# JaredWinkens/sdr-iq-visualizer

Measured on AMD Instinct MI355X. Metric: complex64 IQ Msamples/s through windowed FFT+log-PSD, N=4096; % HBM3E peak, higher is better.
Workload: dtype f32

## Files before the change

### sdr-iq-visualizer_amd/csrc/fft4096.hip

```cpp
#include "fft4096_core.h"

namespace sdrk {

template <bool HAS_WINDOW, int EPILOGUE>
__global__ __launch_bounds__(F4K_THREADS, F4K_WAVES) void fft4096_kernel(
    const float2* __restrict__ iq, size_t frame_stride, void* __restrict__ out_raw,
    size_t n_frames, const float* __restrict__ window, const float2* __restrict__ tw4096,
    float eps, int shift) {
    typedef F4kInC64 In;
    __shared__ float2 lds[f4k_lds_elems(HAS_WINDOW)];
    float2* __restrict__ tw256 = lds + F4K_XCH_ELEMS;
    float2* __restrict__ tw1 = tw256 + 256;
    float* __restrict__ lds_win = reinterpret_cast<float*>(tw1 + 256);

    const int tid = threadIdx.x;
    F4kAddr A = f4k_addr(tid);
    f4k_init_tables(tw256, tw1, tw4096, tid);
    if (HAS_WINDOW) {
#pragma unroll
        for (int j = 0; j < 16; ++j) lds_win[tid + 256 * j] = window[tid + 256 * j];
    }
    __syncthreads();

    const int xor_k2 = shift ? 8 : 0;
    constexpr int OUT_ELEM = (EPILOGUE == EPI_LOGPSD ? 4 : 8);
    const int voff_out = tid * OUT_ELEM;

    const size_t first = blockIdx.x;
    const size_t step = gridDim.x;

    auto issue = [&](In::word (&x)[16], size_t fr) {
        if (fr >= n_frames) fr = first;
        In::issue(x, iq + fr * frame_stride, tid);
    };
    auto process = [&](In::word (&x)[16], size_t f) {
        In::to_owners(x, lds, tid);
        cf v[16];
#pragma unroll
        for (int j = 0; j < 16; ++j) v[j] = In::widen(x[j]);
        issue(x, f + step);
        f4k_windowed_transform<HAS_WINDOW>(v, lds, tw256, tw1, lds_win, A, tid);
        f4k_store_row<EPILOGUE>(v, frame_rsrc(static_cast<char*>(out_raw) + f * (size_t)(F4K_N * OUT_ELEM), F4K_N * OUT_ELEM),
                                voff_out, xor_k2, eps);
    };
    In::word nxt[16];
    issue(nxt, first);
    for (size_t f = first; f < n_frames; f += step) process(nxt, f);
}

hipError_t launch_fft4096(const LaunchArgs& a) {
    if (a.n_frames == 0) return hipSuccess;
    dim3 g(f4k_grid(a.num_cus, F4K_WAVES, a.n_frames)), b(F4K_THREADS);
    const float2* iq = static_cast<const float2*>(a.d_iq);
    const float2* tw = static_cast<const float2*>(a.d_twiddle);
#define SDRK_LAUNCH(W, E)                                                                            \
    hipLaunchKernelGGL((fft4096_kernel<W, E>), g, b, 0, a.stream, iq, a.frame_stride, a.d_out,           \
                       a.n_frames, a.d_window, tw, a.eps, a.shift)
    if (a.epilogue == EPI_LOGPSD) {
        if (a.d_window) SDRK_LAUNCH(true, EPI_LOGPSD); else SDRK_LAUNCH(false, EPI_LOGPSD);
    } else {
        if (a.d_window) SDRK_LAUNCH(true, EPI_COMPLEX); else SDRK_LAUNCH(false, EPI_COMPLEX);
    }
#undef SDRK_LAUNCH
    return hipGetLastError();
}

}
```

### sdr-iq-visualizer_amd/csrc/kernels.h

```cpp
#pragma once
#include <hip/hip_runtime.h>
#include <stddef.h>
#include <stdint.h>

#include <atomic>

#ifdef SDRK_PHASE_MARKS
#define SDRK_PHASE(name) asm volatile("; SDRK_PHASE " name ::: "memory")
#else
#define SDRK_PHASE(name) do { } while (0)
#endif

namespace sdrk {

enum Epilogue : int {
    EPI_LOGPSD = 0,
    EPI_COMPLEX = 1,
    EPI_BLU_MUL = 2,
    EPI_BLU_POST_LOG = 3,
    EPI_BLU_POST_C64 = 4,
};

struct LaunchArgs {
    const void* d_iq = nullptr;
    size_t frame_stride = 0;
    void* d_out = nullptr;
    size_t n_frames = 0;
    int nfft = 0;
    const float* d_window = nullptr;
    const void* d_twiddle = nullptr;
    float eps = 1e-12f;
    int shift = 1;
    int epilogue = EPI_LOGPSD;
    hipStream_t stream = nullptr;
    int num_cus = 256;
    void* d_scratch = nullptr;
    size_t scratch_frames = 0;
    const void* d_twiddle_2p = nullptr;
    hipStream_t stream2 = nullptr;
    hipEvent_t ev_col[2] = {nullptr, nullptr}, ev_row[2] = {nullptr, nullptr}, ev_fork = nullptr;
    int col_cus = 0, row_cus = 0;
    float* d_mip = nullptr;
    bool* mip_written = nullptr;
    const float2* d_epi_tab = nullptr;
    int epi_n_out = 0;
    size_t in_valid = 0;
};

#ifdef __HIPCC__
__device__ __forceinline__ float logpsd_db(float re, float im, float eps) {
    float p = fmaf(re, re, im * im);
    float mag = __builtin_amdgcn_sqrtf(p);
    return __builtin_amdgcn_logf(mag + eps) * 6.02059991327962390427f;
}

__device__ __forceinline__ float logpsd_db_fast(float p) {
    return __builtin_amdgcn_logf(p) * 3.01029995663981195213f;
}

#endif

inline hipError_t ensure_dynamic_lds(const void* kernel, size_t lds_bytes, std::atomic<uint64_t>& mask) {
    if (lds_bytes <= 64 * 1024) return hipSuccess;
    int dev = 0;
    hipError_t e = hipGetDevice(&dev);
    if (e != hipSuccess) return e;
    const uint64_t bit = (dev >= 0 && dev < 64) ? (uint64_t)1 << dev : 0;
    if (bit && (mask.load(std::memory_order_acquire) & bit)) return hipSuccess;
    e = hipFuncSetAttribute(kernel, hipFuncAttributeMaxDynamicSharedMemorySize, (int)lds_bytes);
    if (e == hipSuccess && bit) mask.fetch_or(bit, std::memory_order_release);
    return e;
}

hipError_t launch_fft4096(const LaunchArgs& a);
hipError_t launch_fft_small(const LaunchArgs& a);
bool fft_lds_supports(int nfft);
hipError_t launch_fft_lds(const LaunchArgs& a);
bool fft_tiled2_split(int nfft, int* log2a, int* log2m);
hipError_t launch_fft_tiled2(const LaunchArgs& a);
bool fft_tiled2_has_mip(int nfft, int epilogue);
hipError_t launch_synth_fill(uint32_t seed, uint64_t first_frame, size_t n_frames, int nfft,
                             void* d_iq, hipStream_t stream);

size_t fused64k_ring_bytes();
size_t fused64k_ctrl_words();
unsigned fused64k_sets(int num_cus);
hipError_t launch_fused64k(const LaunchArgs& a, void* d_ring, unsigned* d_ctrl);
bool blu_fused_supports(int M);
hipError_t launch_blu_fused(const void* d_iq, size_t frame_stride, size_t n_frames, int N, int M, const float* d_window,
                            const void* d_chirp, const void* d_bspec, const void* d_twM, float eps, int shift,
                            int epilogue, void* d_out, int num_cus, hipStream_t s);
hipError_t launch_blu_pre(const void* d_iq, size_t frame_stride, size_t n_frames, int N, int M, const float* d_window,
                          const void* d_chirp, void* d_a, int num_cus, hipStream_t s, bool compact = false);
hipError_t launch_blu_mul(const void* d_A, const void* d_B, size_t n_frames, int M, void* d_out, int num_cus,
                          hipStream_t s);
hipError_t launch_blu_post(const void* d_Y, const void* d_chirp, size_t n_frames, int N, int M, float eps, int shift,
                           int epilogue, void* d_out, int num_cus, hipStream_t s);
hipError_t launch_row_features(const float* d_rows, size_t n_rows, int nfft, int rank, float gamma, int min_distance,
                               int max_peaks, double* d_stats, double* d_thr, int* d_idx, int* d_cnt, int num_cus,
                               hipStream_t s);
hipError_t launch_feature_finalize(const double* d_stats, const double* d_thr, const int* d_idx, const int* d_cnt,
                                   size_t n_rows, int nfft, float gamma, int max_peaks, const double* d_freqs,
                                   double* d_out, hipStream_t s);
hipError_t launch_fft4096_features(const LaunchArgs& a, int rank, float gamma, int min_distance, int max_peaks,
                                   double* d_stats, double* d_thr, int* d_idx, int* d_cnt);
hipError_t launch_row_peaks(const float* d_rows, size_t n_rows, int nfft, const double* d_thr, int min_distance,
                            int max_peaks, int* d_idx, int* d_count, hipStream_t s);
hipError_t launch_decimate_rows(const float* d_ring, int nfft, int maxlen, int start_slot, int n_rows, int factor,
                                int mode, float* d_out, hipStream_t stream);
hipError_t launch_decimate_mip(const float* d_mip_ring, int nfft, int maxlen, int start_slot, int n_rows, int factor,
                               float* d_out, hipStream_t stream);
hipError_t launch_stream_mix(const void* d_in, void* d_out, size_t n_frames4096, int num_cus, hipStream_t stream);
hipError_t launch_copy_1to1(const void* d_in, void* d_out, size_t bytes, int num_cus, int blocks_per_cu, hipStream_t stream);
hipError_t launch_power_mean(const void* d_spec, size_t n_frames, int nfft, float scale, float* d_out,
                             hipStream_t stream);

}
```

### sdr-iq-visualizer_amd/csrc/plan_internal.h

```cpp
#pragma once
#include <hip/hip_runtime.h>

#include <cstddef>
#include <cstdint>
#include <map>
#include <mutex>
#include <utility>
#include <vector>

#include "../../include/sdrk.h"
#include "kernels.h"

namespace sdrk_host {
constexpr int HOST_SLOTS = 3;
struct ChunkOut {
    enum Rows {
        None,
        Pooled,
        Direct,
        Kernel,
        Planes,
    } rows = None;
    void* user = nullptr;
    size_t bytes = 0;
// ... 3 lines not shown
    void *h_in = nullptr, *h_out = nullptr;
    void *d_in = nullptr, *d_out = nullptr;
    size_t in_cap = 0, out_cap = 0;
    hipEvent_t ev_in = nullptr, ev_k = nullptr, ev_done = nullptr;
    bool busy = false;
    ChunkOut out;
};

struct Staging {
    hipEvent_t ev = nullptr;
    hipStream_t last = nullptr;
    bool busy = false;
    struct Buf {
        void* d = nullptr;
        size_t cap = 0;
    } buf[2];
    int reserve(int i, size_t need);
    int wait();
    int enter(hipStream_t stream);
    int leave(hipStream_t stream, int st);
    void release();
};
}

struct sdrk_plan {
    int device = 0;
    int nfft = 0;
    size_t max_batch = 0;
    float eps = 1e-12f;
    int shift = 1;
    int num_cus = 256;
    hipStream_t stream = nullptr;
    hipEvent_t ev0 = nullptr, ev1 = nullptr;
    float* d_window = nullptr;
    float2* d_twiddle = nullptr;
    float2* d_scratch = nullptr;
    size_t scratch_frames = 0;
    void* d_in = nullptr;
    size_t in_cap = 0;
    void* d_out = nullptr;
    size_t out_cap = 0;
    void* d_feat = nullptr;
    size_t feat_cap = 0;
    float2* d_tw_2p = nullptr;
    bool tiled2 = false;
    hipStream_t stream2 = nullptr;
    hipEvent_t ev_col[2] = {nullptr, nullptr}, ev_row[2] = {nullptr, nullptr}, ev_fork = nullptr;
    int col_cus = 0, row_cus = 0;
    sdrk_host::HostSlot slot[sdrk_host::HOST_SLOTS];
    float staging_probe_ms[sdrk_host::HOST_SLOTS * 3] = {};
    int staging_probe_n = 0;
    hipStream_t s_h2d = nullptr, s_d2h = nullptr;
    sdrk_plan* blu_inner = nullptr;
    int blu_m = 0;
    float2* d_blu_chirp = nullptr;
    float2* d_blu_bspec = nullptr;
    float2* d_blu_a = nullptr;
    float2* d_blu_b = nullptr;
    size_t blu_frames = 0;
    void* h_small_in = nullptr;
    void* h_small_out = nullptr;
    uint32_t* h_small_flag = nullptr;
    void* d_small_flag = nullptr;
    uint32_t small_seq = 0;
    bool fused64k = false, fused_auto = false, fused_broken = false;
    void* d_fused_ring = nullptr;
    unsigned* d_fused_ctrl = nullptr;
    unsigned* h_fused_err = nullptr;
    unsigned fused_launches = 0, fused_pending = 0;
    int precision = 32;
    double eps64 = 0.0;
    double* d_window64 = nullptr;
    double* d_tw64 = nullptr;
    void* d_scratch64 = nullptr;
    sdrk_host::Staging ci16;
    sdrk_host::Staging integ;
    float* d_pfb_h = nullptr;
    int pfb_taps = 0;
    int pfb_assign = 0;
    sdrk_host::Staging pfb;
    float2* d_fir_h = nullptr;
    int fir_taps = 0;
    int fir_assign = 0;
};

namespace sdrk_host {

constexpr size_t SMALL_IN_BYTES = 256 << 10;
constexpr size_t HOST_CHUNK_BYTES = 16 << 20;
constexpr size_t ZERO_COPY_MAX_BYTES = 32 << 20;
constexpr unsigned FUSED_MAILBOX = 64;
constexpr size_t FUSED_AUTO_MIN_FRAMES = 512;

int fail(int status, const char* fmt, ...) __attribute__((format(printf, 2, 3)));

#define HIP_TRY(expr)                                                                                                   \
    do {                                                                                                                \
        hipError_t e__ = (expr);                                                                                        \
        if (e__ != hipSuccess)                                                                                          \
            return ::sdrk_host::fail(e__ == hipErrorOutOfMemory ? SDRK_ERR_NOMEM : SDRK_ERR_HIP,                        \
                                     "%s failed: %s (%s:%d)", #expr, hipGetErrorString(e__), __FILE__, __LINE__);       \
    } while (0)

int check_device(int device);
bool is_pow2(long long v);

struct PinnedRanges {
    std::mutex m;
    std::map<uintptr_t, std::pair<size_t, bool>> r;
    bool covers(const void* p, size_t bytes) {
        if (!p || bytes == 0) return false;
        std::lock_guard<std::mutex> g(m);
        const uintptr_t a = reinterpret_cast<uintptr_t>(p);
        auto it = r.upper_bound(a);
        if (it == r.begin()) return false;
        --it;
        return a >= it->first && a + bytes <= it->first + it->second.first;
    }
};
PinnedRanges& pinned_ranges();

int grow(int device, void** buf, size_t* cap, size_t need);

inline int Staging::wait() {
    if (busy) {
        HIP_TRY(hipEventSynchronize(ev));
        busy = false;
    }
    return SDRK_OK;
}

inline int Staging::reserve(int i, size_t need) {
    if (!ev) HIP_TRY(hipEventCreateWithFlags(&ev, hipEventDisableTiming));
    Buf& b = buf[i];
    if (need <= b.cap) return SDRK_OK;
    if (int st = wait(); st != SDRK_OK) return st;
    if (b.d) {
        HIP_TRY(hipFree(b.d));
        b.d = nullptr;
        b.cap = 0;
    }
    HIP_TRY(hipMalloc(&b.d, need));
    b.cap = need;
    return SDRK_OK;
}

inline int Staging::enter(hipStream_t stream) {
    if (busy && last != stream) HIP_TRY(hipStreamWaitEvent(stream, ev, 0));
    return SDRK_OK;
}

inline int Staging::leave(hipStream_t stream, int st) {
    const hipError_t e = hipEventRecord(ev, stream);
    last = stream;
    busy = true;
    if (st == SDRK_OK && e != hipSuccess) st = fail(SDRK_ERR_HIP, "hipEventRecord failed: %s", hipGetErrorString(e));
    return st;
}

inline void Staging::release() {
    for (Buf& b : buf)
        if (b.d) (void)hipFree(b.d);
    if (ev) (void)hipEventDestroy(ev);
}

int check_precision(const sdrk_plan* p, int precision);
// ... 132 lines not shown
```

### sdr-iq-visualizer_amd/csrc/sdrk_plan.hip

```cpp
#include "../../include/sdrk.h"

#include <hip/hip_runtime.h>

#include <cmath>
#include <cstdio>
#include <cstdlib>
#include <cstring>
#include <dlfcn.h>
#include <mutex>
#include <new>
#include <vector>

#include "f4k_split.h"
#include "kernels.h"
#include "plan_internal.h"

using namespace sdrk_host;

namespace sdrk_host {

struct EpiArgs {
    const float2* tab = nullptr;
    int n_out = 0;
    float eps = 0.0f;
// ... 56 lines not shown
}

int plan_launch(sdrk_plan* p, const void* d_iq, size_t n_frames, size_t frame_stride, void* d_out,
                int epilogue, hipStream_t stream, float* d_mip, bool* mip_written, const EpiArgs* epi, size_t call_frames) {
    if (p->precision != 32) return fail(SDRK_ERR_INVALID, "float32 transform requested of a float64 plan");
    RoctxRange range(p, n_frames, frame_stride, epilogue);
    if (mip_written) *mip_written = false;
    return plan_launch_impl(p, d_iq, n_frames, frame_stride, d_out, epilogue, stream, d_mip, mip_written, epi,
                            call_frames > n_frames ? call_frames : n_frames);
}

namespace {

int plan_launch_impl(sdrk_plan* p, const void* d_iq, size_t n_frames, size_t frame_stride, void* d_out,
                     int epilogue, hipStream_t stream, float* d_mip, bool* mip_written, const EpiArgs* epi, size_t call_frames) {
    sdrk::LaunchArgs a = plan_launch_args(p, d_iq, n_frames, frame_stride, d_out, epilogue, stream);
    a.d_mip = d_mip;
    a.mip_written = mip_written;
    a.d_scratch = p->d_scratch;
    a.scratch_frames = p->scratch_frames;
    a.d_twiddle_2p = p->d_tw_2p;
    if (epi) {
        if (!p->tiled2 || p->stream2 || epilogue < sdrk::EPI_BLU_MUL)
            return fail(SDRK_ERR_INVALID, "chirp-z epilogues need a serial two-pass inner plan");
        a.d_epi_tab = epi->tab;
        a.epi_n_out = epi->n_out;
        a.eps = epi->eps;
        a.shift = epi->shift;
        a.in_valid = epi->in_valid;
    } else if (epilogue >= sdrk::EPI_BLU_MUL) {
        return fail(SDRK_ERR_INVALID, "epilogue %d needs its table", epilogue);
    }
    if (p->col_cus > 0 && p->stream2) {
        a.stream2 = p->stream2;
        a.ev_fork = p->ev_fork;
        for (int h = 0; h < 2; ++h) { a.ev_col[h] = p->ev_col[h]; a.ev_row[h] = p->ev_row[h]; }
        a.col_cus = p->col_cus;
        a.row_cus = p->row_cus;
    }
    hipError_t e = hipSuccess;
    if (p->blu_inner) {
        const int N = p->nfft, M = p->blu_m;
        const size_t out_elem = epilogue == sdrk::EPI_LOGPSD ? sizeof(float) : sizeof(float2);
        for (size_t f0 = 0; f0 < n_frames; f0 += p->blu_frames) {
            const size_t nf = n_frames - f0 < p->blu_frames ? n_frames - f0 : p->blu_frames;
            if (sdrk::blu_fused_supports(M)) {
                e = sdrk::launch_blu_fused(static_cast<const float2*>(d_iq) + f0 * frame_stride, frame_stride, nf, N, M,
                                           p->d_window, p->d_blu_chirp, p->d_blu_bspec, p->blu_inner->d_twiddle,
                                           p->eps, p->shift, epilogue,
                                           static_cast<char*>(d_out) + f0 * (size_t)N * out_elem, p->num_cus, stream);
                if (e != hipSuccess) break;
                continue;
            }
            const bool fused_multiplies = p->blu_inner->tiled2 && !p->blu_inner->stream2;
            e = sdrk::launch_blu_pre(static_cast<const float2*>(d_iq) + f0 * frame_stride, frame_stride, nf, N, M,
                                     p->d_window, p->d_blu_chirp, p->d_blu_a, p->num_cus, stream, fused_multiplies);
            if (e != hipSuccess) break;
            if (fused_multiplies) {
                EpiArgs mul, post;
                mul.tab = p->d_blu_bspec;
                mul.in_valid = (size_t)N;
                post.tab = p->d_blu_chirp;
                post.n_out = N;
                post.eps = p->eps;
                post.shift = p->shift;
                int st = plan_launch(p->blu_inner, p->d_blu_a, nf, (size_t)M, p->d_blu_b, sdrk::EPI_BLU_MUL, stream, nullptr, nullptr, &mul);
                if (st != SDRK_OK) return st;
                st = plan_launch(p->blu_inner, p->d_blu_b, nf, (size_t)M, static_cast<char*>(d_out) + f0 * (size_t)N * out_elem,
                                 epilogue == sdrk::EPI_LOGPSD ? sdrk::EPI_BLU_POST_LOG : sdrk::EPI_BLU_POST_C64, stream, nullptr, nullptr, &post);
                if (st != SDRK_OK) return st;
                continue;
            }
            int st = plan_launch(p->blu_inner, p->d_blu_a, nf, (size_t)M, p->d_blu_b, sdrk::EPI_COMPLEX, stream);
            if (st != SDRK_OK) return st;
            e = sdrk::launch_blu_mul(p->d_blu_b, p->d_blu_bspec, nf, M, p->d_blu_a, p->num_cus, stream);
            if (e != hipSuccess) break;
            st = plan_launch(p->blu_inner, p->d_blu_a, nf, (size_t)M, p->d_blu_b, sdrk::EPI_COMPLEX, stream);
            if (st != SDRK_OK) return st;
            e = sdrk::launch_blu_post(p->d_blu_b, p->d_blu_chirp, nf, N, M, p->eps, p->shift, epilogue,
                                      static_cast<char*>(d_out) + f0 * (size_t)N * out_elem, p->num_cus, stream);
            if (e != hipSuccess) break;
        }
    } else if (p->nfft == 4096) {
        const size_t parts = f4k_split_parts(n_frames);
        const size_t per = (n_frames + parts - 1) / parts;
        const size_t out_elem = epilogue == sdrk::EPI_LOGPSD ? sizeof(float) : sizeof(float2);
        for (size_t f0 = 0; f0 < n_frames && e == hipSuccess; f0 += per) {
            a.d_iq = static_cast<const float2*>(d_iq) + f0 * frame_stride;
            a.d_out = static_cast<char*>(d_out) + f0 * (size_t)4096 * out_elem;
            a.n_frames = n_frames - f0 < per ? n_frames - f0 : per;
            e = sdrk::launch_fft4096(a);
        }
    } else if (sdrk::fft_lds_supports(p->nfft))
        e = sdrk::launch_fft_lds(a);
    else if (p->nfft < 4096)
        e = sdrk::launch_fft_small(a);
    else if (takes_fused(p, call_frames) && !d_mip && epilogue <= sdrk::EPI_COMPLEX) {
        FusedGate& gate = fused_gate(p->device);
        std::lock_guard<std::mutex> lk(gate.mu);
        if (gate.ev && gate.last_stream != stream && gate.recorded) e = hipStreamWaitEvent(stream, gate.ev, 0);
        if (e == hipSuccess) e = sdrk::launch_fused64k(a, p->d_fused_ring, p->d_fused_ctrl);
        if (e == hipSuccess)
            e = hipMemcpyAsync(p->h_fused_err + 16 * (p->fused_launches++ % FUSED_MAILBOX), p->d_fused_ctrl,
                               16 * sizeof(unsigned), hipMemcpyDeviceToHost, stream);
        if (e == hipSuccess && gate.ev) {
            e = hipEventRecord(gate.ev, stream);
            gate.last_stream = stream;
            gate.recorded = true;
        }
        ++p->fused_pending;
    } else if (p->tiled2)
        e = sdrk::launch_fft_tiled2(a);
    else
        return fail(SDRK_ERR_UNSUPPORTED, "no kernel for nfft=%d", p->nfft);
    if (e != hipSuccess) return fail(SDRK_ERR_HIP, "kernel launch failed: %s", hipGetErrorString(e));
    return SDRK_OK;
}

RoctxRange::RoctxRange(const sdrk_plan* p, size_t n_frames, size_t stride, int epilogue) {
    Roctx& r = roctx();
    if (!r.push) return;
    char label[160];
    snprintf(label, sizeof label, "sdrk.plan_launch nfft=%d frames=%zu stride=%zu %s dev=%d", p->nfft, n_frames, stride,
             epilogue == sdrk::EPI_LOGPSD ? "logpsd" : (epilogue == sdrk::EPI_COMPLEX ? "complex" : "chirp-z stage"), p->device);
    r.push(label);
    on = true;
}
RoctxRange::~RoctxRange() {
    if (on) roctx().pop();
}

}

int fused_check(sdrk_plan* p) {
    if (!p->h_fused_err || p->fused_pending == 0) return SDRK_OK;
    const unsigned want = sdrk::fused64k_sets(p->num_cus);
    unsigned bad = 0, rec[16] = {0};
    const unsigned pending = p->fused_pending < FUSED_MAILBOX ? p->fused_pending : FUSED_MAILBOX;
    for (unsigned k = 0; k < pending; ++k) {
        const unsigned* r = p->h_fused_err + 16 * ((p->fused_launches - 1 - k) % FUSED_MAILBOX);
        const unsigned code = r[1] ? r[1] : (r[0] != want ? 9u : 0u);
        if (code) { memcpy(rec, r, sizeof rec); bad = code; }
    }
    p->fused_pending = 0;
    if (bad && p->fused_auto) p->fused_broken = true;
    if (bad)
        return fail(SDRK_ERR_HIP, "fused N=65536 kernel reported an internal synchronisation error (code %u; %u of %u sets formed; "
                    "word %u held %u, wanted %u, site %u)", bad, rec[0], want, rec[2], rec[3], rec[4], rec[5]);
    return SDRK_OK;
}

int check_precision(const sdrk_plan* p, int precision) {
    if (p->precision == precision) return SDRK_OK;
    return fail(SDRK_ERR_INVALID, "this is a float%d plan (sdrk_plan_create%s) and the call is a float%d entry point%s",
                p->precision, p->precision == 64 ? "_f64" : "", precision,
                precision == 64 ? " (sdrk_*_f64)" : ": use the sdrk_*_f64 entry points");
}

int check_exec_args(const sdrk_plan* p, const void* in, size_t n_frames, size_t frame_stride,
                    const void* out, int precision) {
    if (!p) return fail(SDRK_ERR_INVALID, "plan is NULL");
    if (int st = check_precision(p, precision); st != SDRK_OK) return st;
    if (n_frames == 0) return SDRK_OK;
    if (!in || !out) return fail(SDRK_ERR_INVALID, "input or output pointer is NULL");
    if (frame_stride == 0 && n_frames > 1)
        return fail(SDRK_ERR_INVALID, "frame_stride must be >= 1 for more than one frame");
    return SDRK_OK;
}

int check_exec_f32(const sdrk_plan* p, const void* in, size_t n_frames, size_t frame_stride, const void* out) {
    return check_exec_args(p, in, n_frames, frame_stride, out, 32);
}

}
// ... 34 lines not shown
    if (st != SDRK_OK) return st;
    HIP_TRY(hipSetDevice(device));
    hipDeviceProp_t prop;
    HIP_TRY(hipGetDeviceProperties(&prop, device));
    if (strncmp(prop.gcnArchName, "gfx950", 6) != 0)
        return fail(SDRK_ERR_NO_DEVICE, "device %d is %s; this library is built for gfx950 only",
                    device, prop.gcnArchName);

    sdrk_plan* p = new (std::nothrow) sdrk_plan();
    if (!p) return fail(SDRK_ERR_NOMEM, "out of host memory");
    p->device = device;
    p->nfft = nfft;
    p->max_batch = max_batch;
    p->eps = eps;
    p->shift = shift ? 1 : 0;
    p->num_cus = prop.multiProcessorCount > 0 ? prop.multiProcessorCount : 256;
    if (const char* env = getenv("SDRK_NUM_CUS")) {
        long v = atol(env);
        if (v >= 1 && v < p->num_cus) p->num_cus = (int)v;
    }

#define PLAN_TRY(expr)                                                                     \
    do {                                                                                   \
        hipError_t e__ = (expr);                                                           \
        if (e__ != hipSuccess) {                                                           \
            int s__ = fail(e__ == hipErrorOutOfMemory ? SDRK_ERR_NOMEM : SDRK_ERR_HIP,     \
                           "%s failed: %s", #expr, hipGetErrorString(e__));                \
            sdrk_plan_destroy(p);                                                          \
            return s__;                                                                    \
        }                                                                                  \
    } while (0)

    PLAN_TRY(hipStreamCreateWithFlags(&p->stream, hipStreamNonBlocking));
    PLAN_TRY(hipEventCreate(&p->ev0));
    PLAN_TRY(hipEventCreate(&p->ev1));

    if (window_kind != SDRK_WINDOW_RECT) {
        std::vector<float> w(nfft);
        if (window_kind == SDRK_WINDOW_HANN) {
            for (int n = 0; n < nfft; ++n)
                w[n] = (float)(0.5 - 0.5 * std::cos(2.0 * M_PI * (double)n / (double)(nfft - 1)));
        } else {
            memcpy(w.data(), window, sizeof(float) * nfft);
        }
        PLAN_TRY(hipMalloc((void**)&p->d_window, sizeof(float) * nfft));
        PLAN_TRY(hipMemcpy(p->d_window, w.data(), sizeof(float) * nfft, hipMemcpyHostToDevice));
    }
    if (!is_pow2(nfft)) {
        int M = 1;
        while (M < 2 * nfft - 1) M <<= 1;
        p->blu_m = M;
        const bool one_kernel = sdrk::blu_fused_supports(M);
        size_t frames = ((size_t)128 << 20) / ((size_t)M * sizeof(float2));
        if (frames < 1) frames = 1;
        if (frames > max_batch || one_kernel) frames = max_batch;
        p->blu_frames = frames;
        int st2 = sdrk_plan_create(device, M, frames, SDRK_WINDOW_RECT, nullptr, 0.0f, 0, &p->blu_inner);
        if (st2 != SDRK_OK) { sdrk_plan_destroy(p); return st2; }
        std::vector<float2> c(nfft), b(M, make_float2(0.f, 0.f));
        for (long long n = 0; n < nfft; ++n) {
            const long long r = (n * n) % (2LL * nfft);
            const double ang = M_PI * (double)r / (double)nfft;
            c[n] = make_float2((float)std::cos(ang), (float)std::sin(ang));
            b[n] = c[n];
            if (n) b[M - n] = c[n];
        }
        PLAN_TRY(hipMalloc((void**)&p->d_blu_chirp, sizeof(float2) * nfft));
        PLAN_TRY(hipMemcpy(p->d_blu_chirp, c.data(), sizeof(float2) * nfft, hipMemcpyHostToDevice));
        PLAN_TRY(hipMalloc((void**)&p->d_blu_a, (one_kernel ? 1 : frames) * (size_t)M * sizeof(float2)));
        if (!one_kernel) PLAN_TRY(hipMalloc((void**)&p->d_blu_b, frames * (size_t)M * sizeof(float2)));
        PLAN_TRY(hipMalloc((void**)&p->d_blu_bspec, (size_t)M * sizeof(float2)));
        PLAN_TRY(hipMemcpy(p->d_blu_a, b.data(), sizeof(float2) * M, hipMemcpyHostToDevice));
        st2 = plan_launch(p->blu_inner, p->d_blu_a, 1, (size_t)M, p->d_blu_bspec, sdrk::EPI_COMPLEX, p->stream);
        if (st2 != SDRK_OK) { sdrk_plan_destroy(p); return st2; }
        PLAN_TRY(hipStreamSynchronize(p->stream));
        *out = p;
        return SDRK_OK;
    }
    if (nfft <= 16384) {
        std::vector<float2> t(nfft);
        for (int m = 0; m < nfft; ++m) t[m] = twiddle(m, nfft);
        PLAN_TRY(hipMalloc((void**)&p->d_twiddle, sizeof(float2) * nfft));
        PLAN_TRY(hipMemcpy(p->d_twiddle, t.data(), sizeof(float2) * nfft, hipMemcpyHostToDevice));
    } else {
        size_t scratch_mb = 192;
        if (const char* env = getenv("SDRK_SCRATCH_MB")) {
            long v = atol(env);
            if (v >= 1 && v <= 65536) scratch_mb = (size_t)v;
        }
        size_t frames = (scratch_mb << 20) / ((size_t)nfft * sizeof(float2));
        if (frames < 1) frames = 1;
        if (frames > max_batch) frames = max_batch;
        p->scratch_frames = frames;
        PLAN_TRY(hipMalloc((void**)&p->d_scratch, frames * (size_t)nfft * sizeof(float2)));
        int la = 0, lm = 0;
        if (!sdrk::fft_tiled2_split(nfft, &la, &lm)) {
            sdrk_plan_destroy(p);
            return fail(SDRK_ERR_UNSUPPORTED, "no kernel for nfft=%d", nfft);
        }
        const int A = 1 << la, M = 1 << lm, TA = A / 16;
        std::vector<float2> t((size_t)4096 + (size_t)TA * M + (size_t)M * 16);
        for (int m = 0; m < A; ++m) t[m] = twiddle(m, A);
        for (int m = 0; m < M; ++m) t[2048 + m] = twiddle(m, M);
        for (int tau = 0; tau < TA; ++tau)
            for (int m = 0; m < M; ++m) t[4096 + (size_t)tau * M + m] = twiddle((double)m * tau, (double)nfft);
        for (int m = 0; m < M; ++m)
            for (int q = 0; q < 16; ++q)
                t[4096 + (size_t)TA * M + (size_t)m * 16 + q] = twiddle((double)m * TA * q, (double)nfft);
        PLAN_TRY(hipMalloc((void**)&p->d_tw_2p, sizeof(float2) * t.size()));
        PLAN_TRY(hipMemcpy(p->d_tw_2p, t.data(), sizeof(float2) * t.size(), hipMemcpyHostToDevice));
        p->tiled2 = true;
        if (flags & SDRK_PLAN_OVERLAP_PASSES) {
            PLAN_TRY(hipStreamCreateWithFlags(&p->stream2, hipStreamNonBlocking));
            PLAN_TRY(hipEventCreateWithFlags(&p->ev_fork, hipEventDisableTiming));
            for (int h = 0; h < 2; ++h) {
                PLAN_TRY(hipEventCreateWithFlags(&p->ev_col[h], hipEventDisableTiming));
                PLAN_TRY(hipEventCreateWithFlags(&p->ev_row[h], hipEventDisableTiming));
            }
            p->col_cus = p->num_cus * 3 / 4 > 0 ? p->num_cus * 3 / 4 : 1;
            p->row_cus = p->num_cus / 2 > 0 ? p->num_cus / 2 : 1;
            if (const char* c = getenv("SDRK_OVL_COL_CUS")) { long v = atol(c); if (v >= 1 && v <= 4096) p->col_cus = (int)v; }
            if (const char* c = getenv("SDRK_OVL_ROW_CUS")) { long v = atol(c); if (v >= 1 && v <= 4096) p->row_cus = (int)v; }
        }
    }
    const bool fused_auto = nfft == 65536 && !(flags & (SDRK_PLAN_FUSED64K | SDRK_PLAN_TILED64K | SDRK_PLAN_OVERLAP_PASSES)) &&
                            p->num_cus >= 32 && p->num_cus % 32 == 0;
    if ((flags & SDRK_PLAN_FUSED64K) || fused_auto) {
        p->fused64k = (flags & SDRK_PLAN_FUSED64K) != 0;
        p->fused_auto = fused_auto;
        PLAN_TRY(hipMalloc(&p->d_fused_ring, sdrk::fused64k_ring_bytes()));
        PLAN_TRY(hipMalloc((void**)&p->d_fused_ctrl, sdrk::fused64k_ctrl_words() * sizeof(unsigned)));
        PLAN_TRY(hipHostMalloc((void**)&p->h_fused_err, FUSED_MAILBOX * 16 * sizeof(unsigned), hipHostMallocDefault));
        memset(p->h_fused_err, 0, FUSED_MAILBOX * 16 * sizeof(unsigned));
    }
#undef PLAN_TRY
    if (flags & SDRK_PLAN_TUNE_STAGING) {
        st = tune_staging(p);
        if (st != SDRK_OK) { sdrk_plan_destroy(p); return st; }
    }
    *out = p;
    return SDRK_OK;
}

int sdrk_plan_staging_probe(const sdrk_plan* p, float* probe_ms, int capacity, int* n) {
    if (!p || !n) return fail(SDRK_ERR_INVALID, "plan or n is NULL");
    *n = p->staging_probe_n;
    for (int i = 0; i < p->staging_probe_n && i < capacity && probe_ms; ++i) probe_ms[i] = p->staging_probe_ms[i];
    return SDRK_OK;
}

int sdrk_plan_fused_status(const sdrk_plan* p, unsigned* launches, int* fallen_back) {
    if (!p) return fail(SDRK_ERR_INVALID, "plan is NULL");
    if (launches) *launches = p->fused_launches;
    if (fallen_back) *fallen_back = p->fused_broken ? 1 : 0;
    return SDRK_OK;
}

int sdrk_plan_destroy(sdrk_plan* p) {
    if (!p) return SDRK_OK;
    (void)hipSetDevice(p->device);
    if (p->stream) (void)hipStreamSynchronize(p->stream);
    if (p->stream2) { (void)hipStreamSynchronize(p->stream2); (void)hipStreamDestroy(p->stream2); }
    if (p->ev_fork) (void)hipEventDestroy(p->ev_fork);
    for (int h = 0; h < 2; ++h) {
        if (p->ev_col[h]) (void)hipEventDestroy(p->ev_col[h]);
        if (p->ev_row[h]) (void)hipEventDestroy(p->ev_row[h]);
    }
    if (p->d_window) (void)hipFree(p->d_window);
    if (p->d_window64) (void)hipFree(p->d_window64);
    if (p->d_tw64) (void)hipFree(p->d_tw64);
    if (p->d_scratch64) (void)hipFree(p->d_scratch64);
    if (p->d_twiddle) (void)hipFree(p->d_twiddle);
    if (p->d_tw_2p) (void)hipFree(p->d_tw_2p);
    if (p->d_scratch) (void)hipFree(p->d_scratch);
    if (p->blu_inner) (void)sdrk_plan_destroy(p->blu_inner);
    if (p->d_blu_chirp) (void)hipFree(p->d_blu_chirp);
    if (p->d_blu_bspec) (void)hipFree(p->d_blu_bspec);
    if (p->d_blu_a) (void)hipFree(p->d_blu_a);
    if (p->d_blu_b) (void)hipFree(p->d_blu_b);
    if (p->h_small_in) (void)hipHostFree(p->h_small_in);
    if (p->h_small_out) (void)hipHostFree(p->h_small_out);
    if (p->h_small_flag) (void)hipHostFree(p->h_small_flag);
    if (p->d_fused_ring) (void)hipFree(p->d_fused_ring);
    if (p->d_fused_ctrl) (void)hipFree(p->d_fused_ctrl);
    if (p->h_fused_err) (void)hipHostFree(p->h_fused_err);
    if (p->d_in) (void)hipFree(p->d_in);
    if (p->d_out) (void)hipFree(p->d_out);
    if (p->d_feat) (void)hipFree(p->d_feat);
    p->ci16.release();
    p->integ.release();
    if (p->d_pfb_h) (void)hipFree(p->d_pfb_h);
    p->pfb.release();
    if (p->d_fir_h) (void)hipFree(p->d_fir_h);
    if (p->s_h2d) (void)hipStreamSynchronize(p->s_h2d);
    if (p->s_d2h) (void)hipStreamSynchronize(p->s_d2h);
    for (auto& sl : p->slot) {
        if (sl.h_in) (void)hipHostFree(sl.h_in);
        if (sl.h_out) (void)hipHostFree(sl.h_out);
        if (sl.d_in) (void)hipFree(sl.d_in);
        if (sl.d_out) (void)hipFree(sl.d_out);
        if (sl.ev_in) (void)hipEventDestroy(sl.ev_in);
        if (sl.ev_k) (void)hipEventDestroy(sl.ev_k);
        if (sl.ev_done) (void)hipEventDestroy(sl.ev_done);
    }
    if (p->s_h2d) (void)hipStreamDestroy(p->s_h2d);
    if (p->s_d2h) (void)hipStreamDestroy(p->s_d2h);
    if (p->ev0) (void)hipEventDestroy(p->ev0);
    if (p->ev1) (void)hipEventDestroy(p->ev1);
    if (p->stream) (void)hipStreamDestroy(p->stream);
    delete p;
    return SDRK_OK;
}

int sdrk_plan_nfft(const sdrk_plan* p) { return p ? p->nfft : fail(SDRK_ERR_INVALID, "plan is NULL"); }
int sdrk_plan_device(const sdrk_plan* p) { return p ? p->device : fail(SDRK_ERR_INVALID, "plan is NULL"); }

int sdrk_exec_device(sdrk_plan* p, const void* d_iq, size_t n_frames, size_t frame_stride,
                     float* d_out_db, void* stream) {
    return exec_device_frames(check_exec_f32, launch_f32, p, d_iq, n_frames, frame_stride, d_out_db, stream);
}

int sdrk_plan_sync(sdrk_plan* p) {
    if (!p) return fail(SDRK_ERR_INVALID, "plan is NULL");
    HIP_TRY(hipSetDevice(p->device));
    HIP_TRY(hipStreamSynchronize(p->stream));
    return fused_check(p);
}

int sdrk_exec_device_timed(sdrk_plan* p, const void* d_iq, size_t n_frames, size_t frame_stride,
                           float* d_out_db, int launches, float* elapsed_ms) {
    if (!elapsed_ms || launches < 1) return fail(SDRK_ERR_INVALID, "bad launches/elapsed_ms");
    int st = check_exec_args(p, d_iq, n_frames, frame_stride, d_out_db);
    if (st != SDRK_OK) return st;
    HIP_TRY(hipSetDevice(p->device));
    HIP_TRY(hipEventRecord(p->ev0, p->stream));
    for (int i = 0; i < launches; ++i) {
        st = plan_launch(p, d_iq, n_frames, frame_stride, d_out_db, sdrk::EPI_LOGPSD, p->stream);
        if (st != SDRK_OK) return st;
    }
    HIP_TRY(hipEventRecord(p->ev1, p->stream));
    HIP_TRY(hipEventSynchronize(p->ev1));
    HIP_TRY(hipEventElapsedTime(elapsed_ms, p->ev0, p->ev1));
    return fused_check(p);
}

int sdrk_exec_device_timed_each(sdrk_plan* p, const void* d_iq, size_t n_frames, size_t frame_stride,
                                float* d_out_db, int launches, float* each_ms) {
    return exec_device_frames_timed_each(check_exec_f32, launch_f32, p, d_iq, n_frames, frame_stride, d_out_db, launches, each_ms);
}

}
```

Measured before the change: 499,200.

## Add atomic ticket-based dynamic frame scheduling for the 4096-point FFT kernel

Adds a persistent FFT4096 kernel variant where workgroups draw frame tickets from a global atomic counter, in pairs of frames per ticket with draws prefetched a few tickets ahead, instead of a fixed grid-stride assignment. It is enabled by default when the frame count is at least the maximum block count and that count is a multiple of eight, and it launches the whole batch as one part instead of splitting. The intent is to keep workgroups progressing together through memory, reducing the lag between the leading and trailing frames and the tail imbalance, so HBM access stays more sequential. In exchange it adds atomics per ticket, persistent head counters with base bookkeeping across launches, and a cross-stream event wait, plus an optional timeline instrumentation build and analysis script.

```diff
diff --git a/experiments/f4k_order/timeline.py b/experiments/f4k_order/timeline.py
--- /dev/null
+++ b/experiments/f4k_order/timeline.py
@@ -0,0 +1,100 @@
+import argparse
+import ctypes
+import json
+import os
+import sys
+
+REPO = os.path.dirname(os.path.dirname(os.path.dirname(os.path.abspath(__file__))))
+sys.path.insert(0, REPO)
+import torch
+import numpy as np
+from bench import warm_up_by_time
+from sdr_iq_visualizer_amd import _ffi
+from sdr_iq_visualizer_amd.spectrum import SpectrumPlan
+
+NFFT = 4096
+TICK_NS = 10.0
+BIN_MS = 0.5
+
+
+def analyse(rec, n_frames):
+    t = rec[:, 0].astype(np.uint64) | (rec[:, 1].astype(np.uint64) << np.uint64(32))
+    assert (t > 0).all(), "frames without a record"
+    assert np.array_equal(rec[:, 2], np.arange(n_frames, dtype=np.uint32)), "a record names another frame than its own"
+    wg = rec[:, 3].astype(np.int64)
+    grid = int(wg.max()) + 1
+    ms = (t - t.min()).astype(np.float64) * TICK_NS * 1e-6
+    frame = np.arange(n_frames, dtype=np.int64)
+    last_ms = np.zeros(grid)
+    np.maximum.at(last_ms, wg, ms)
+    order = np.argsort(ms, kind="stable")
+    bins = []
+    reached = np.full(grid, -1, dtype=np.int64)
+    n_bins = int(np.ceil((ms.max() + 1e-9) / BIN_MS))
+    cut = np.searchsorted(ms[order], np.arange(n_bins + 1) * BIN_MS, side="left")
+    cut[-1] = n_frames
+    for b in range(n_bins):
+        hi = (b + 1) * BIN_MS
+        idx = order[cut[b]:cut[b + 1]]
+        if idx.size == 0:
+            continue
+        reached[wg[idx]] = frame[idx]
+        active = (last_ms >= hi) & (reached >= 0)
+        front = int(reached.max())
+        lag = int(front - reached[active].min()) if active.any() else 0
+        bins.append({"ms": round(b * BIN_MS, 2), "frames": int(idx.size), "span": int(frame[idx].max() - frame[idx].min()),
+                     "lag_frames": lag, "lag_grids": round(lag / grid, 2)})
+    return {"grid": grid, "launch_ms_by_records": round(float(ms.max()), 3), "bins": bins}
+
+
+def main():
+    ap = argparse.ArgumentParser()
+    ap.add_argument("--out", required=True)
+    ap.add_argument("--frames", type=int, default=1 << 20)
+    ap.add_argument("--short", type=int, default=65536)
+    ap.add_argument("--pairs", type=int, default=3)
+    a = ap.parse_args()
+    lib = _ffi.lib()
+    _ffi.require_device(0)
+    set_tl = lib.sdrk_f4k_timeline
+    set_tl.argtypes, set_tl.restype = [ctypes.c_void_p], ctypes.c_int
+    os.environ["SDRK_F4K_PARTS"] = "1"
+    d_in = ctypes.c_void_p()
+    _ffi.check(lib.sdrk_dev_alloc(0, a.frames * NFFT * 8, ctypes.byref(d_in)))
+    outs = []
+    for _ in range(a.pairs):
+        p = ctypes.c_void_p()
+        _ffi.check(lib.sdrk_dev_alloc(0, a.frames * NFFT * 4, ctypes.byref(p)))
+        outs.append(p)
+    _ffi.check(lib.sdrk_synth_fill(0, 1234, 0, a.frames, NFFT, d_in, None))
+    tl = torch.zeros((a.frames, 4), dtype=torch.int32, device="cuda")
+    os.makedirs(os.path.dirname(os.path.abspath(a.out)), exist_ok=True)
+    with open(a.out, "a") as out:
+        for order in ("stride", "ticket"):
+            os.environ["SDRK_F4K_ORDER"] = order
+            with SpectrumPlan(NFFT, window="hann", device=0) as plan:
+                warm_up_by_time(lambda: plan.exec_device_timed(d_in.value, a.frames, outs[0].value, 1))
+                for i, p in enumerate(outs):
+                    for n in (a.frames, a.short):
+                        plan.exec_device_timed(d_in.value, n, p.value, 1)
+                        tl.zero_()
+                        torch.cuda.synchronize()
+                        assert set_tl(tl.data_ptr()) == 0
+                        ms = plan.exec_device_timed(d_in.value, n, p.value, 1)
+                        assert set_tl(None) == 0
+                        rec = tl[:n].cpu().numpy().view(np.uint32)
+                        r = {"order": order, "pair": i, "frames": n, "launch_ms_by_events": round(float(ms), 4), **analyse(rec, n)}
+                        out.write(json.dumps(r) + "\n")
+                        out.flush()
+                        print(f"== {order} pair {i} frames {n}: {r['launch_ms_by_events']} ms by events, "
+                              f"{r['launch_ms_by_records']} ms first to last issue, grid {r['grid']}")
+                        for b in r["bins"]:
+                            print(f"   {b['ms']:5.2f} ms  frames {b['frames']:7d}  span {b['span']:8d}  lag {b['lag_frames']:8d} "
+                                  f"frames = {b['lag_grids']:7.2f} grids", flush=True)
+    for p in outs:
+        lib.sdrk_dev_free(0, p)
+    lib.sdrk_dev_free(0, d_in)
+
+
+if __name__ == "__main__":
+    main()
diff --git a/sdr-iq-visualizer_amd/csrc/f4k_ticket.h b/sdr-iq-visualizer_amd/csrc/f4k_ticket.h
--- /dev/null
+++ b/sdr-iq-visualizer_amd/csrc/f4k_ticket.h
@@ -0,0 +1,61 @@
+#pragma once
+#include <cstddef>
+#include <cstdint>
+
+namespace sdrk_host {
+
+constexpr unsigned F4K_TICKET_MAX_HEADS = 8;
+constexpr unsigned F4K_TICKET_HEAD_WORDS = 32;
+constexpr size_t F4K_TICKET_MAX_FRAMES = (size_t)1 << 31;
+
+struct F4kTicketForm {
+    unsigned heads;
+    unsigned frames;
+};
+constexpr bool f4k_ticket_form_ok(F4kTicketForm f) {
+    return f.heads >= 1 && f.heads <= F4K_TICKET_MAX_HEADS && !(f.heads & (f.heads - 1)) && f.frames >= 1 && f.frames <= 8 &&
+           !(f.frames & (f.frames - 1));
+}
+constexpr F4kTicketForm F4K_TICKET_FORM = {1, 2};
+
+enum F4kOrder { F4K_ORDER_AUTO = 0, F4K_ORDER_STRIDE = 1, F4K_ORDER_TICKET = 2 };
+
+struct F4kTicketBases {
+    uint32_t base[F4K_TICKET_MAX_HEADS];
+};
+
+constexpr unsigned f4k_ticket_depth(F4kTicketForm f) { return f.frames == 1 ? 4 : 3; }
+constexpr size_t f4k_ticket_first_frame(F4kTicketForm f, uint32_t ticket, unsigned head) {
+    return ((size_t)ticket * f.heads + head) * f.frames;
+}
+constexpr size_t f4k_ticket_draws(F4kTicketForm f, size_t n_frames) { return f.frames == 1 ? n_frames : (n_frames + 1) / f.frames; }
+constexpr size_t f4k_ticket_class(F4kTicketForm f, size_t n_frames, unsigned head) {
+    return (f4k_ticket_draws(f, n_frames) + f.heads - 1 - head) / f.heads;
+}
+constexpr unsigned f4k_ticket_pullers(F4kTicketForm f, unsigned grid, unsigned head) { return (grid + f.heads - 1 - head) / f.heads; }
+
+constexpr unsigned f4k_ticket_grid(size_t max_blocks, size_t n_frames) {
+    if (max_blocks < F4K_TICKET_MAX_HEADS || n_frames == 0 || n_frames > F4K_TICKET_MAX_FRAMES) return 0;
+    const size_t full = max_blocks - max_blocks % F4K_TICKET_MAX_HEADS;
+    const size_t need = (n_frames + F4K_TICKET_MAX_HEADS - 1) / F4K_TICKET_MAX_HEADS * F4K_TICKET_MAX_HEADS;
+    return (unsigned)(need < full ? need : full);
+}
+
+constexpr uint32_t f4k_ticket_advance(F4kTicketForm f, uint32_t base, size_t n_frames, unsigned grid, unsigned head) {
+    return base + (uint32_t)f4k_ticket_class(f, n_frames, head) + f4k_ticket_depth(f) * f4k_ticket_pullers(f, grid, head);
+}
+inline void f4k_ticket_advance(F4kTicketForm f, F4kTicketBases& b, size_t n_frames, unsigned grid) {
+    for (unsigned x = 0; x < f.heads; ++x) b.base[x] = f4k_ticket_advance(f, b.base[x], n_frames, grid, x);
+}
+
+constexpr bool f4k_ticket_takes(int order, size_t max_blocks, size_t n_frames, bool by_default) {
+    if (order == F4K_ORDER_STRIDE || f4k_ticket_grid(max_blocks, n_frames) == 0) return false;
+    if (order == F4K_ORDER_TICKET) return true;
+    return by_default && n_frames >= max_blocks && max_blocks % F4K_TICKET_MAX_HEADS == 0;
+}
+
+constexpr bool F4K_TICKET_DEFAULT = true;
+
+constexpr size_t f4k_ticket_parts(size_t) { return 1; }
+
+}
diff --git a/sdr-iq-visualizer_amd/csrc/fft4096.hip b/sdr-iq-visualizer_amd/csrc/fft4096.hip
--- a/sdr-iq-visualizer_amd/csrc/fft4096.hip
+++ b/sdr-iq-visualizer_amd/csrc/fft4096.hip
@@ -1,6 +1,21 @@
 #include "fft4096_core.h"
 
 namespace sdrk {
+
+#ifdef SDRK_F4K_TIMELINE
+__device__ uint4* f4k_timeline_buf = nullptr;
+#define F4K_TIMELINE_LOAD() uint4* const f4k_tl = f4k_timeline_buf
+#define F4K_TIMELINE_MARK(fr)                                                                                   \
+    do {                                                                                                        \
+        if (f4k_tl && tid == 0 && (fr) < n_frames) {                                                            \
+            const unsigned long long f4k_t = wall_clock64();                                                    \
+            f4k_tl[fr] = make_uint4((unsigned)f4k_t, (unsigned)(f4k_t >> 32), (unsigned)(fr), blockIdx.x);      \
+        }                                                                                                       \
+    } while (0)
+#else
+#define F4K_TIMELINE_LOAD() (void)0
+#define F4K_TIMELINE_MARK(fr) (void)0
+#endif
 
 template <bool HAS_WINDOW, int EPILOGUE>
 __global__ __launch_bounds__(F4K_THREADS, F4K_WAVES) void fft4096_kernel(
@@ -28,8 +43,10 @@
 
     const size_t first = blockIdx.x;
     const size_t step = gridDim.x;
+    F4K_TIMELINE_LOAD();
 
     auto issue = [&](In::word (&x)[16], size_t fr) {
+        F4K_TIMELINE_MARK(fr);
         if (fr >= n_frames) fr = first;
         In::issue(x, iq + fr * frame_stride, tid);
     };
@@ -48,6 +65,83 @@
     for (size_t f = first; f < n_frames; f += step) process(nxt, f);
 }
 
+template <bool HAS_WINDOW, int EPILOGUE>
+__global__ __launch_bounds__(F4K_THREADS, F4K_WAVES) void fft4096_ticket_kernel(
+    const float2* __restrict__ iq, size_t frame_stride, void* __restrict__ out_raw,
+    size_t n_frames, const float* __restrict__ window, const float2* __restrict__ tw4096,
+    float eps, int shift, unsigned* __restrict__ heads, const sdrk_host::F4kTicketBases bases,
+    const sdrk_host::F4kTicketForm form) {
+    typedef F4kInC64 In;
+    __shared__ float2 lds[f4k_lds_elems(HAS_WINDOW)];
+    __shared__ unsigned ticket_slot[2];
+    float2* __restrict__ tw256 = lds + F4K_XCH_ELEMS;
+    float2* __restrict__ tw1 = tw256 + 256;
+    float* __restrict__ lds_win = reinterpret_cast<float*>(tw1 + 256);
+
+    const int tid = threadIdx.x;
+    const unsigned hx = blockIdx.x & (form.heads - 1);
+    const unsigned depth = sdrk_host::f4k_ticket_depth(form);
+    unsigned* const head = heads + hx * sdrk_host::F4K_TICKET_HEAD_WORDS + __lane_id();
+    const unsigned base = bases.base[hx];
+    unsigned drawn = 0;
+    if (tid == 0) drawn = __hip_atomic_fetch_add(head, depth, __ATOMIC_RELAXED, __HIP_MEMORY_SCOPE_AGENT);
+    F4kAddr A = f4k_addr(tid);
+    f4k_init_tables(tw256, tw1, tw4096, tid);
+    if (HAS_WINDOW) {
+#pragma unroll
+        for (int j = 0; j < 16; ++j) lds_win[tid + 256 * j] = window[tid + 256 * j];
+    }
+    if (tid == 0) {
+        ticket_slot[0] = drawn;
+        drawn += depth - 1;
+    }
+    __syncthreads();
+
+    const int xor_k2 = shift ? 8 : 0;
+    constexpr int OUT_ELEM = (EPILOGUE == EPI_LOGPSD ? 4 : 8);
+    const int voff_out = tid * OUT_ELEM;
+    F4K_TIMELINE_LOAD();
+
+    auto first_of = [&](unsigned head_value) { return sdrk_host::f4k_ticket_first_frame(form, head_value - base, hx); };
+    const unsigned h0 = __builtin_amdgcn_readfirstlane(ticket_slot[0]);
+    const size_t in_ticket = form.frames - 1;
+    size_t cur = first_of(h0), nx = in_ticket ? cur + 1 : first_of(h0 + 1), tn = first_of(h0 + depth - 2);
+    unsigned par = 1;
+
+    auto issue = [&](In::word (&x)[16], size_t fr) {
+        F4K_TIMELINE_MARK(fr);
+        if (fr >= n_frames) fr = 0;
+        In::issue(x, iq + fr * frame_stride, tid);
+    };
+    In::word nxt[16];
+    issue(nxt, cur);
+    while (cur < n_frames) {
+        const bool last_of_ticket = ((nx + 1) & in_ticket) == 0;
+        if (last_of_ticket && tid == 0) {
+            ticket_slot[par] = drawn;
+            drawn = __hip_atomic_fetch_add(head, 1u, __ATOMIC_RELAXED, __HIP_MEMORY_SCOPE_AGENT);
+        }
+        In::to_owners(nxt, lds, tid);
+        cf v[16];
+#pragma unroll
+        for (int j = 0; j < 16; ++j) v[j] = In::widen(nxt[j]);
+        issue(nxt, nx);
+        f4k_windowed_transform<HAS_WINDOW>(v, lds, tw256, tw1, lds_win, A, tid);
+        size_t after = nx + 1;
+        if (last_of_ticket) {
+            after = tn;
+            tn = first_of(__builtin_amdgcn_readfirstlane(ticket_slot[par]));
+            par ^= 1;
+        }
+        f4k_store_row<EPILOGUE>(v, frame_rsrc(static_cast<char*>(out_raw) + cur * (size_t)(F4K_N * OUT_ELEM), F4K_N * OUT_ELEM),
+                                voff_out, xor_k2, eps);
+        cur = nx;
+        nx = after;
+    }
+}
+
+unsigned f4k_max_blocks(int num_cus) { return f4k_grid(num_cus, F4K_WAVES, (size_t)-1); }
+
 hipError_t launch_fft4096(const LaunchArgs& a) {
     if (a.n_frames == 0) return hipSuccess;
     dim3 g(f4k_grid(a.num_cus, F4K_WAVES, a.n_frames)), b(F4K_THREADS);
@@ -65,4 +159,30 @@
     return hipGetLastError();
 }
 
+hipError_t launch_fft4096_ticket(const LaunchArgs& a, unsigned* d_heads, const sdrk_host::F4kTicketBases& bases,
+                                 sdrk_host::F4kTicketForm form, unsigned grid) {
+    if (a.n_frames == 0) return hipSuccess;
+    if (!d_heads || grid == 0 || grid % sdrk_host::F4K_TICKET_MAX_HEADS || !sdrk_host::f4k_ticket_form_ok(form)) return hipErrorInvalidValue;
+    dim3 g(grid), b(F4K_THREADS);
+    const float2* iq = static_cast<const float2*>(a.d_iq);
+    const float2* tw = static_cast<const float2*>(a.d_twiddle);
+#define SDRK_LAUNCH(W, E)                                                                            \
+    hipLaunchKernelGGL((fft4096_ticket_kernel<W, E>), g, b, 0, a.stream, iq, a.frame_stride, a.d_out,    \
+                       a.n_frames, a.d_window, tw, a.eps, a.shift, d_heads, bases, form)
+    if (a.epilogue == EPI_LOGPSD) {
+        if (a.d_window) SDRK_LAUNCH(true, EPI_LOGPSD); else SDRK_LAUNCH(false, EPI_LOGPSD);
+    } else {
+        if (a.d_window) SDRK_LAUNCH(true, EPI_COMPLEX); else SDRK_LAUNCH(false, EPI_COMPLEX);
+    }
+#undef SDRK_LAUNCH
+    return hipGetLastError();
 }
+
+}
+
+#ifdef SDRK_F4K_TIMELINE
+extern "C" int sdrk_f4k_timeline(void* d_records) {
+    uint4* p = static_cast<uint4*>(d_records);
+    return (int)hipMemcpyToSymbol(HIP_SYMBOL(sdrk::f4k_timeline_buf), &p, sizeof p);
+}
+#endif
diff --git a/sdr-iq-visualizer_amd/csrc/kernels.h b/sdr-iq-visualizer_amd/csrc/kernels.h
--- a/sdr-iq-visualizer_amd/csrc/kernels.h
+++ b/sdr-iq-visualizer_amd/csrc/kernels.h
@@ -4,6 +4,8 @@
 #include <stdint.h>
 
 #include <atomic>
+
+#include "f4k_ticket.h"
 
 #ifdef SDRK_PHASE_MARKS
 #define SDRK_PHASE(name) asm volatile("; SDRK_PHASE " name ::: "memory")
@@ -73,6 +75,9 @@
 }
 
 hipError_t launch_fft4096(const LaunchArgs& a);
+unsigned f4k_max_blocks(int num_cus);
+hipError_t launch_fft4096_ticket(const LaunchArgs& a, unsigned* d_heads, const sdrk_host::F4kTicketBases& bases,
+                                 sdrk_host::F4kTicketForm form, unsigned grid);
 hipError_t launch_fft_small(const LaunchArgs& a);
 bool fft_lds_supports(int nfft);
 hipError_t launch_fft_lds(const LaunchArgs& a);
diff --git a/sdr-iq-visualizer_amd/csrc/plan_internal.h b/sdr-iq-visualizer_amd/csrc/plan_internal.h
--- a/sdr-iq-visualizer_amd/csrc/plan_internal.h
+++ b/sdr-iq-visualizer_amd/csrc/plan_internal.h
@@ -109,6 +109,14 @@
     float2* d_fir_h = nullptr;
     int fir_taps = 0;
     int fir_assign = 0;
+    int f4k_order = sdrk_host::F4K_ORDER_AUTO;
+    sdrk_host::F4kTicketForm f4k_form = sdrk_host::F4K_TICKET_FORM;
+    unsigned* d_f4k_heads = nullptr;
+    sdrk_host::F4kTicketBases f4k_bases = {};
+    hipEvent_t f4k_ev = nullptr;
+    hipStream_t f4k_last = nullptr;
+    bool f4k_recorded = false;
+    size_t f4k_parts = 0;
 };
 
 namespace sdrk_host {
diff --git a/sdr-iq-visualizer_amd/csrc/sdrk_plan.hip b/sdr-iq-visualizer_amd/csrc/sdrk_plan.hip
--- a/sdr-iq-visualizer_amd/csrc/sdrk_plan.hip
+++ b/sdr-iq-visualizer_amd/csrc/sdrk_plan.hip
@@ -162,14 +162,29 @@
             if (e != hipSuccess) break;
         }
     } else if (p->nfft == 4096) {
-        const size_t parts = f4k_split_parts(n_frames);
+        const size_t max_blocks = sdrk::f4k_max_blocks(p->num_cus);
+        const bool ticket = p->d_f4k_heads && f4k_ticket_takes(p->f4k_order, max_blocks, n_frames, F4K_TICKET_DEFAULT);
+        size_t parts = p->f4k_parts ? p->f4k_parts : (ticket ? f4k_ticket_parts(n_frames) : f4k_split_parts(n_frames));
+        if (p->f4k_parts && parts > n_frames) parts = n_frames ? n_frames : 1;
         const size_t per = (n_frames + parts - 1) / parts;
         const size_t out_elem = epilogue == sdrk::EPI_LOGPSD ? sizeof(float) : sizeof(float2);
+        if (ticket && p->f4k_recorded && p->f4k_last != stream) e = hipStreamWaitEvent(stream, p->f4k_ev, 0);
         for (size_t f0 = 0; f0 < n_frames && e == hipSuccess; f0 += per) {
             a.d_iq = static_cast<const float2*>(d_iq) + f0 * frame_stride;
             a.d_out = static_cast<char*>(d_out) + f0 * (size_t)4096 * out_elem;
             a.n_frames = n_frames - f0 < per ? n_frames - f0 : per;
-            e = sdrk::launch_fft4096(a);
+            if (ticket) {
+                const unsigned grid = f4k_ticket_grid(max_blocks, a.n_frames);
+                e = sdrk::launch_fft4096_ticket(a, p->d_f4k_heads, p->f4k_bases, p->f4k_form, grid);
+                if (e == hipSuccess) f4k_ticket_advance(p->f4k_form, p->f4k_bases, a.n_frames, grid);
+            } else {
+                e = sdrk::launch_fft4096(a);
+            }
+        }
+        if (ticket && e == hipSuccess) {
+            e = hipEventRecord(p->f4k_ev, stream);
+            p->f4k_last = stream;
+            p->f4k_recorded = true;
         }
     } else if (sdrk::fft_lds_supports(p->nfft))
         e = sdrk::launch_fft_lds(a);
@@ -370,6 +385,23 @@
         for (int m = 0; m < nfft; ++m) t[m] = twiddle(m, nfft);
         PLAN_TRY(hipMalloc((void**)&p->d_twiddle, sizeof(float2) * nfft));
         PLAN_TRY(hipMemcpy(p->d_twiddle, t.data(), sizeof(float2) * nfft, hipMemcpyHostToDevice));
+        if (nfft == 4096) {
+            if (const char* env = getenv("SDRK_F4K_ORDER"))
+                p->f4k_order = env[0] == 't' ? F4K_ORDER_TICKET : (env[0] == 's' ? F4K_ORDER_STRIDE : F4K_ORDER_AUTO);
+            if (const char* env = getenv("SDRK_F4K_PARTS")) {
+                long v = atol(env);
+                if (v >= 1 && v <= 4096) p->f4k_parts = (size_t)v;
+            }
+            if (const char* env = getenv("SDRK_F4K_TICKET_FORM")) {
+                F4kTicketForm f = {0, 0};
+                if (sscanf(env, "%ux%u", &f.heads, &f.frames) == 2 && f4k_ticket_form_ok(f)) p->f4k_form = f;
+            }
+            std::vector<uint32_t> h(F4K_TICKET_MAX_HEADS * F4K_TICKET_HEAD_WORDS, 0u);
+            for (unsigned x = 0; x < F4K_TICKET_MAX_HEADS; ++x) h[x * F4K_TICKET_HEAD_WORDS] = p->f4k_bases.base[x] = 0xFFFFFE00u;
+            PLAN_TRY(hipMalloc((void**)&p->d_f4k_heads, h.size() * sizeof(uint32_t)));
+            PLAN_TRY(hipMemcpy(p->d_f4k_heads, h.data(), h.size() * sizeof(uint32_t), hipMemcpyHostToDevice));
+            PLAN_TRY(hipEventCreateWithFlags(&p->f4k_ev, hipEventDisableTiming));
+        }
     } else {
         size_t scratch_mb = 192;
         if (const char* env = getenv("SDRK_SCRATCH_MB")) {
@@ -480,6 +512,9 @@
     if (p->d_pfb_h) (void)hipFree(p->d_pfb_h);
     p->pfb.release();
     if (p->d_fir_h) (void)hipFree(p->d_fir_h);
+    if (p->f4k_recorded) (void)hipEventSynchronize(p->f4k_ev);
+    if (p->d_f4k_heads) (void)hipFree(p->d_f4k_heads);
+    if (p->f4k_ev) (void)hipEventDestroy(p->f4k_ev);
     if (p->s_h2d) (void)hipStreamSynchronize(p->s_h2d);
     if (p->s_d2h) (void)hipStreamSynchronize(p->s_d2h);
     for (auto& sl : p->slot) {
```

New measurement: 517,300, median of 6. +3.6%, better.
